# TheRealOrange/icer_compression

Hardware: AMD Instinct MI355X
Metric: Mpixels/s encode (bit-exact), 4096x4096 gray (higher is better)
Workload: dtype int16

## Files before the change

### icer_compression_amd/csrc/api.hip

```cpp
#include <hip/hip_runtime.h>

#include <algorithm>
#include <atomic>
#include <map>
#include <memory>
#include <mutex>
#include <thread>
#include <sched.h>
#include <time.h>
#include <stdarg.h>
#include <stdio.h>
#include <stdlib.h>
#include <string.h>
#include <string>
#include <vector>

#include "../../include/icer_hip.h"
#include "kernels.hpp"
#include "launch_plan.hpp"
#include "subband_gain.hpp"

using namespace icer;

namespace {
// ... 425 lines not shown
    return hipSuccess;
}
const char *pool_compute_level() { const char *v = getenv("ICER_HIP_COMPUTE_LEVEL"); return v ? v : "low"; }

#ifndef ICER_LONE_PAD_BYTES
#define ICER_LONE_PAD_BYTES 12288
#endif
constexpr int kLonePadBytes = ICER_LONE_PAD_BYTES;
static_assert(kUnitWavesSmall == 8 && kUnitWavesLarge == 11, "launch_plan.hpp names the pipeline's shapes by these wave counts");

int enqueue_budget_tail(icerx_encoder *e, const EncodeCall &c)
{
    const Budget &b = *c.budget;
    const uint32_t n_units = (uint32_t)e->plan.units.size();
    const size_t off_pitch = (size_t)e->max_frames * n_units, curve_pitch = (size_t)n_units + 1u;
    hipLaunchKernelGGL(budget_search_kernel, dim3(b.n), dim3(64 * kBudgetWaves), 0, c.stream, e->curve.p, e->curve.p + (size_t)e->max_frames * curve_pitch,
                       e->curve_head.p, n_units, (uint32_t)b.n_frames, b.budgets, (uint64_t)c.quota, e->unit_bits.p, e->final_order.p, e->skip(0), e->units.p,
                       e->final_off.p, off_pitch, reinterpret_cast<unsigned long long *>(c.d_sizes), c.d_rcs, b.d_at_cap, b.d_dist, b.d_equiv, b.d_threshold,
                       b.d_total, e->bound_ovf(), e->budget_state.p);
    hipLaunchKernelGGL(gather_ladder_kernel, dim3(n_units, b.n_frames), dim3(256), 0, c.stream, e->slots.p, e->plan.slot_bytes, e->units.p, n_units,
                       e->unit_bits.p, e->final_off.p, off_pitch, (uint32_t)b.n, c.d_out, c.out_stride, (uint32_t)b.n_frames);
    HIP_TRY(hipGetLastError());
    return 0;
}

int enqueue_part(icerx_encoder *e, const LaunchPlan &lp, int part, bool timed, const EncodeCall &c, bool clear_bound)
{
    const PartPlan &pp = lp.part[part];
    const int f0 = pp.f0, n_frames = pp.n_frames;
    const uint16_t *const d_frames = c.d_frames; uint8_t *const d_out = c.d_out; int32_t *const d_rcs = c.d_rcs;
    unsigned long long *const d_sizes = reinterpret_cast<unsigned long long *>(c.d_sizes);
    const size_t quota = c.quota, out_stride = c.out_stride;
    const hipStream_t st = c.stream; const Ladder *const ladder = c.ladder; const Target *const target = c.target; const Budget *const budget = c.budget;
    const Roi *const roi = c.roi;
    const bool energy = target || budget;
    const bool progressive = lp.progressive, use_wg = lp.use_wg, split = pp.split, hybrid = pp.hybrid;
    const size_t W = e->w, H = e->h, plane = W * H;
    const int C = e->channels, P = n_frames * C;
    const uint32_t n_units = (uint32_t)e->plan.units.size();
    int *dwt_ovf = e->dwt_ovf(f0), *mean_ovf = e->mean_ovf(f0), *skip = e->skip(f0), *bound_ovf = e->bound_ovf();
    int16_t *const coef = e->coef.p + (size_t)f0 * C * plane, *const tmp = e->tmp.p + (size_t)f0 * C * plane;
    unsigned long long *const sums = e->sums.p + (size_t)f0 * C;
    uint16_t *const means = e->means.p + (size_t)f0 * C;
    uint8_t *const sig = e->sig.p + (size_t)f0 * e->plan.sig_bytes;
    uint32_t *const sig_hist = e->sig_hist.p + (size_t)f0 * e->plan.n_families * 16;
    uint8_t *const route_buf = e->route.p + (size_t)f0 * n_units;
    uint32_t *const route_list = e->route_list.p + 2 * (size_t)f0 * n_units,        *const route_ctl = e->route_ctl.p + 4 * (size_t)part;
    uint8_t *const slots = e->slots.p + (size_t)f0 * e->plan.slot_bytes;
    uint32_t *const unit_bits = e->unit_bits.p + (size_t)f0 * n_units, *const done_bytes = e->done_bytes.p + (size_t)f0 * n_units;
    uint64_t *const final_off = e->final_off.p + (size_t)f0 * n_units;
    const size_t sub_entries = e->plan.sub_entries;
    if (split && (e->snaps.ensure((size_t)e->max_frames * sub_entries * kMaxSnaps) || e->snap_valid.ensure((size_t)e->max_frames * sub_entries * kMaxSnaps) ||
                  e->sub_recs.ensure((size_t)e->max_frames * sub_entries))) return ICER_FATAL_ERROR;
    {
        ClearList cl;
        const char *bad = nullptr;
        auto clear = [&](const char *what, void *ptr, size_t bytes) { if (!bad && !cl.add(ptr, bytes)) bad = what; };
        if (f0 == 0 && n_frames == e->max_frames && clear_bound) clear("frame flags", e->flags.p, e->flags.n * sizeof(int));
        else {
            clear("transform flags", dwt_ovf, (size_t)P * sizeof(int)); clear("mean flags", mean_ovf, (size_t)P * sizeof(int)); clear("skip flags", skip, (size_t)n_frames * sizeof(int));
            if (clear_bound) clear("slot bound flag", bound_ovf, sizeof(int));
        }
        clear("LL sums", sums, (size_t)P * sizeof(unsigned long long));
        if (progressive) clear("unit byte counts", done_bytes, (size_t)n_frames * n_units * 4);
        if (hybrid) { clear("chunk histograms", sig_hist, (size_t)n_frames * e->plan.n_families * 16 * sizeof(uint32_t)); clear("route list cursor", route_ctl, 4 * sizeof(uint32_t)); }
        if (split) { clear("snapshot flags", e->snap_valid.p, (size_t)n_frames * sub_entries * kMaxSnaps * sizeof(uint32_t)); clear("sub-range records", e->sub_recs.p, (size_t)n_frames * sub_entries * sizeof(SubRecord)); }
        if (bad) { set_error("enqueue: the clear kernel cannot take the %s range (%d ranges queued)", bad, cl.n); return ICER_FATAL_ERROR; }
        launch_clears(cl, st);
    }
    if (timed && e->timing) HIP_TRY(hipEventRecord(e->ev[0], st));

    size_t cw = W, ch = H;
    launch_dwt(e, d_frames, n_frames, st, e->sample_bits, dwt_ovf, &cw, &ch, coef, tmp);
    if (timed && e->timing) HIP_TRY(hipEventRecord(e->ev[1], st));

    const uint32_t llw = (uint32_t)cw, llh = (uint32_t)ch;
    unsigned sum_blocks = (llw * llh + 255) / 256;
    if (sum_blocks > 64) sum_blocks = 64;
    hipLaunchKernelGGL(ll_sum_kernel, dim3(sum_blocks, P), dim3(256), 0, st, reinterpret_cast<const uint16_t *>(coef),
                       plane, (uint32_t)W, llw, llh, sums, e->sample_bits == 8 ? 0xFFu : 0xFFFFu);
    hipLaunchKernelGGL(ll_mean_kernel, dim3((P + 63) / 64), dim3(64), 0, st, sums, (uint32_t)P, llw * llh,
                       means, mean_ovf, e->sample_bits);
    hipLaunchKernelGGL(frame_status_kernel, dim3((n_frames + 63) / 64), dim3(64), 0, st, dwt_ovf, mean_ovf, C, n_frames, skip);
    hipLaunchKernelGGL(finalize_ll_kernel, dim3((llw + 63u) / 64u, (llh + 3u) / 4u, P), dim3(256), 0, st,
                       reinterpret_cast<uint16_t *>(coef), plane, (uint32_t)W, llw, llh, means, skip, C, e->sample_bits);
    if (timed && e->timing) HIP_TRY(hipEventRecord(e->ev[2], st));
    if (e->coef_ready && f0 == 0) HIP_TRY(hipEventRecord(e->coef_ready, st));

    const int n_planes = e->sample_bits == 8 ? kPlanes8 : kPlanes;
    const size_t ev_frame_bytes = (size_t)n_planes * e->plan.sig_bytes * 64u;
    {
        hipLaunchKernelGGL(family_events_kernel, dim3((unsigned)(e->plan.sig_blocks.size() / 2), n_frames), dim3(256), 0, st,
                           reinterpret_cast<const uint16_t *>(coef), plane, (uint32_t)W, C, e->units.p, e->sig_blocks.p, skip, sig,
                           e->plan.sig_bytes, hybrid ? sig_hist : nullptr, e->plan.n_families,
                           use_wg ? nullptr : e->events.p + (size_t)f0 * ev_frame_bytes, ev_frame_bytes, (uint32_t)n_planes);
    }
    const uint8_t *route = nullptr;
    if (hybrid) {
        hipLaunchKernelGGL(route_units_kernel, dim3((unsigned)((n_units + 255) / 256), n_frames), dim3(256), 0, st, e->units.p, n_units, sig_hist, e->plan.n_families,
                           pp.route_percent, 16u, route_buf, route_list, route_ctl, kNoSplitPercent, (uint32_t)n_frames * n_units, kListHeavyMin);
        route = route_buf;
        HIP_TRY(hipEventRecord(e->fork[part], st));
        HIP_TRY(hipStreamWaitEvent(e->side_stream, e->fork[part], 0));
#define ICER_LAUNCH_LIST(I, NS)                                                                                                          \
        hipLaunchKernelGGL((code_units_list_kernel<I>), dim3(pp.list_grid), dim3(64 * NS::kWgWaves), sizeof(NS::Shared), e->side_stream, \
                           reinterpret_cast<const uint16_t *>(coef), plane, (uint32_t)W, (uint32_t)H, C, e->units.p, n_units,     \
                           e->tables.p, means, skip, slots, e->plan.slot_bytes, unit_bits, sig,                     \
                           e->plan.sig_bytes, route_list, route_ctl, e->prof.p ? e->prof.p + kProfWgsOffset : nullptr, (uint32_t)n_frames * n_units)
        if (pp.list == ListKernel::One) ICER_LAUNCH_LIST(WgOne, wg1); else if (pp.list == ListKernel::Four) ICER_LAUNCH_LIST(WgFour, wg4); else ICER_LAUNCH_LIST(WgSmall, wgs);
#undef ICER_LAUNCH_LIST
        HIP_TRY(hipEventRecord(e->join[part], e->side_stream));
    }
    const uint32_t tgt_planes = (uint32_t)n_planes;
    unsigned long long *const dist = energy ? e->dist.p + (size_t)f0 * e->plan.n_families * (tgt_planes + 1u) : nullptr;
    auto launch_energy = [&](hipStream_t es) -> int {
        HIP_TRY(hipMemsetAsync(dist, 0, (size_t)n_frames * e->plan.n_families * (tgt_planes + 1u) * sizeof(unsigned long long), es));
        hipLaunchKernelGGL(family_energy_kernel, dim3((unsigned)(e->plan.sig_blocks.size() / 2), n_frames), dim3(64 * kEnergyWaves), 0, es,
                           reinterpret_cast<const uint16_t *>(coef), plane, (uint32_t)W, C, e->units.p, e->sig_blocks.p, dist, e->plan.n_families, tgt_planes);
        return 0;
    };
    if (energy && e->side_stream) {
        HIP_TRY(hipEventRecord(e->energy_fork[part], st));
        HIP_TRY(hipStreamWaitEvent(e->side_stream, e->energy_fork[part], 0));
        if (launch_energy(e->side_stream)) return ICER_FATAL_ERROR;
        HIP_TRY(hipEventRecord(e->energy_join[part], e->side_stream));
    }
    SplitLaunch sp;
    if (split) {
        sp.subs = e->subs.p; sp.launch = e->sub_order.p; sp.n_subs = pp.subs; sp.entries = (uint32_t)sub_entries;
        sp.snaps = e->snaps.p; sp.snap_valid = e->snap_valid.p; sp.recs = e->sub_recs.p;
    }
    uint32_t fail_inject = ~0u;
    if (Tuning &t = e->tuning; t.fail_calls > 0 && !use_wg && t.fail_frame >= f0 && t.fail_frame < f0 + n_frames && t.fail_unit < (int)n_units) {
        fail_inject = ((uint32_t)(t.fail_frame - f0) << 20) | (uint32_t)t.fail_unit;
        t.fail_calls--;
    }
    if (!use_wg) {
        const dim3 pipe_grid = pp.position_major ? dim3((unsigned)((n_units + sp.n_subs) * (unsigned)n_frames), 1) : dim3(n_units + sp.n_subs, n_frames);
// ... 1279 lines not shown
```

### icer_compression_amd/csrc/events.hpp

```cpp
#pragma once
#include "icer_tables.hpp"
#include "wave.hpp"

namespace icer {

constexpr uint32_t kEvNone = 14u, kEvUncoded = 15u;

ICER_HD uint32_t ev_ctx_plain(uint32_t h, uint32_t v, uint32_t d)
{
    if (h == 2) return 8;
    if (h == 1) return (v == 0) ? (d < 2 ? 5 + d : 7u) : 7u;
    if (v == 0) return d > 2 ? 2u : d;
    return 2 + v;
}
ICER_HD uint32_t ev_ctx_hh(uint32_t hv, uint32_t d)
{
    if (d >= 3) return 8;
    const uint32_t k = hv > 2 ? 2u : hv;
    if (d == 0) return k;
    if (d == 1) return 3 + k;
    return hv == 0 ? 6u : 7u;
}
ICER_HD uint32_t ev_ctx_entry(bool is_hh, uint32_t i)
{
    return is_hh ? ev_ctx_hh(i / 5u, i % 5u) : ev_ctx_plain(i / 15u, (i / 5u) % 3u, i % 5u);
}

struct PixelLens {
    uint32_t mag;
    uint32_t msb;
    uint32_t aW, aE, aN, aS, aNW, aNE, aSW, aSE;
    uint32_t neg;
    uint32_t t;
};

ICER_HD uint32_t ev_len(uint32_t v) { const uint32_t m = v & 0x7FFFu; return m ? 32u - (uint32_t)__builtin_clz(m) : 0u; }

ICER_HD PixelLens pixel_lens(uint32_t vC, uint32_t vW, uint32_t vE, uint32_t vN, uint32_t vS, uint32_t vNW, uint32_t vNE, uint32_t vSW, uint32_t vSE)
{
    PixelLens L;
    const uint32_t lc = ev_len(vC);
    L.mag = vC & 0x7FFFu;
    L.msb = lc ? lc - 1u : 0u;
    L.aW = ev_len(vW); L.aN = ev_len(vN); L.aNW = ev_len(vNW); L.aNE = ev_len(vNE);
    const uint32_t lE = ev_len(vE), lS = ev_len(vS), lSW = ev_len(vSW), lSE = ev_len(vSE);
    L.aE = lE ? lE - 1u : 0u; L.aS = lS ? lS - 1u : 0u; L.aSW = lSW ? lSW - 1u : 0u; L.aSE = lSE ? lSE - 1u : 0u;
    L.neg = ((vW >> 15) & 1u) | (((vE >> 15) & 1u) << 1) | (((vN >> 15) & 1u) << 2) | (((vS >> 15) & 1u) << 3) | (((vC >> 15) & 1u) << 4);
    uint32_t t = lc;
    t = L.aW > t ? L.aW : t; t = L.aN > t ? L.aN : t; t = L.aNW > t ? L.aNW : t; t = L.aNE > t ? L.aNE : t;
    t = L.aE > t ? L.aE : t; t = L.aS > t ? L.aS : t; t = L.aSW > t ? L.aSW : t; t = L.aSE > t ? L.aSE : t;
    L.t = t;
    return L;
}

ICER_HD uint32_t event_byte(const PixelLens &L, uint32_t p, bool is_hl, bool is_hh, const uint8_t *ctx_tab)
{
    const uint32_t sW = L.aW > p, sE = L.aE > p, sN = L.aN > p, sS = L.aS > p;
    uint32_t hh = sW + sE, vv = sN + sS;
    const uint32_t dd = (uint32_t)(L.aNW > p) + (uint32_t)(L.aNE > p) + (uint32_t)(L.aSW > p) + (uint32_t)(L.aSE > p);
    const uint32_t up = L.msb > p ? L.msb - p : 0u, cat = up > 3u ? 3u : up;
    const uint32_t bit = (L.mag >> p) & 1u;
    uint32_t A = (L.neg & sW) | ((L.neg >> 1) & sE), B = ((L.neg >> 2) & sN) | ((L.neg >> 3) & sS);
    if (is_hl) { uint32_t x = hh; hh = vv; vv = x; x = A; A = B; B = x; }
    const uint32_t c0 = ctx_tab[is_hh ? (hh + vv) * 5u + dd : (hh * 3u + vv) * 5u + dd];
    const uint32_t ctx = cat == 0u ? c0 : cat == 1u ? (hh + vv == 0u ? 9u : 10u) : cat == 2u ? 11u : kEvUncoded;
    const uint32_t s2 = ((A & 1u) << 1) | ((A ^ B) & 1u);
    const uint32_t bit2 = (A ^ (L.neg >> 4)) & 1u;
    return ctx | (bit << 4) | (s2 << 5) | (bit2 << 7);
}

ICER_HD size_t ev_offset(uint32_t p, size_t chunks_per_frame, uint32_t chunk_off, uint32_t j) { return ((size_t)p * chunks_per_frame + chunk_off + j) * 64u; }

}
```

### icer_compression_amd/csrc/kernels.hpp

```cpp
#pragma once
#include <hip/hip_runtime.h>

#include "assemble_core.hpp"
#include "assemble_ladder.hpp"
#include "roi_core.hpp"
#include "coder_core.hpp"
#include "distortion_core.hpp"
#include "budget_core.hpp"
#include "coder_wg.hpp"
#include "coder_wg_small.hpp"
#include "dwt_tile.hpp"
#include "events.hpp"
#include "plan.hpp"

namespace icer {

__global__ void __launch_bounds__(kTileThreads)
dwt_tile_kernel(DwtStageArgs a, size_t src_plane, size_t coef_plane, size_t ll_plane, int *__restrict__ ovf)
{
    __shared__ union { DwtTileShared gen; DwtFastShared fast; } u;
    a.src += blockIdx.z * src_plane;
    a.coef += blockIdx.z * coef_plane;
    a.ll += blockIdx.z * ll_plane;
    const int tx = blockIdx.x, ty = blockIdx.y, t = threadIdx.x;
// ... 6 lines not shown
        __syncthreads();
        o |= dwt_fast_cols_step2(u.fast, a, tx, ty, t);
        if (o) atomicOr(&ovf[blockIdx.z], 1);
        return;
    }
    DwtTileShared &sh = u.gen;
    dwt_tile_load(sh, a, tx, ty, t);
    __syncthreads();
    bool o = dwt_tile_rows_step1(sh, a, tx, ty, t);
    __syncthreads();
    o |= dwt_tile_rows_step2(sh, a, tx, ty, t);
    __syncthreads();
    o |= dwt_tile_cols_step1(sh, a, tx, ty, t);
    __syncthreads();
    o |= dwt_tile_cols_step2(sh, a, tx, ty, t);
    if (o) atomicOr(&ovf[blockIdx.z], 1);
}

__global__ void __launch_bounds__(256)
ll_sum_kernel(const uint16_t *__restrict__ coef, size_t plane, uint32_t stride, uint32_t llw, uint32_t llh,
              unsigned long long *__restrict__ sums, uint32_t mask)
{
    const uint16_t *p = coef + blockIdx.y * plane;
    const uint32_t n = llw * llh;
    unsigned long long acc = 0;
    for (uint32_t i = blockIdx.x * 256 + threadIdx.x; i < n; i += gridDim.x * 256) {
        const uint32_t r = i / llw, c = i - r * llw;
        acc += p[(size_t)r * stride + c] & mask;
    }
    for (int o = 32; o > 0; o >>= 1) acc += __shfl_down(acc, o);
    if ((threadIdx.x & 63) == 0 && acc) atomicAdd(&sums[blockIdx.y], acc);
}

__global__ void ll_mean_kernel(const unsigned long long *__restrict__ sums, uint32_t n_planes, uint32_t ll_count,
                               uint16_t *__restrict__ means, int *__restrict__ mean_ovf, int sample_bits)
{
    const uint32_t p = blockIdx.x * blockDim.x + threadIdx.x;
    if (p >= n_planes) return;
    const uint16_t m = sample_bits == 8 ? (uint16_t)(uint8_t)(sums[p] / ll_count) : (uint16_t)(sums[p] / ll_count);
    means[p] = m;
    mean_ovf[p] = m > (sample_bits == 8 ? 127 : 32767) ? 1 : 0;
}

__global__ void __launch_bounds__(256)
finalize_ll_kernel(uint16_t *__restrict__ coef, size_t plane, uint32_t w, uint32_t llw, uint32_t llh,
                   const uint16_t *__restrict__ means, const int *__restrict__ frame_skip, int channels, int sample_bits)
{
    const uint32_t c = blockIdx.x * 64 + (threadIdx.x & 63), r = blockIdx.y * 4 + (threadIdx.x >> 6);
    if (c >= llw || r >= llh) return;
    if (frame_skip[blockIdx.z / channels]) return;
    uint16_t *q = coef + blockIdx.z * plane + (size_t)r * w + c;
    const int16_t v = (int16_t)((int16_t)*q - (int16_t)means[blockIdx.z]);
    *q = (uint16_t)to_coder_word(v, sample_bits);
}

struct SplitLaunch {
    const SubDesc *subs = nullptr;
    const uint32_t *launch = nullptr;
    uint32_t n_subs = 0;
    uint32_t entries = 0;
    Snapshot *snaps = nullptr;
    uint32_t *snap_valid = nullptr;
    SubRecord *recs = nullptr;
};

constexpr uint8_t kRoutePipeline = 0, kRouteWindows = 1, kRouteNoSplit = 2;

template <int WAVES, int OCC, int LDS_PAD>
__global__ void __launch_bounds__(64 * WAVES, OCC)
code_units_kernel(const uint16_t *__restrict__ coef, size_t plane, uint32_t img_w, uint32_t img_h, int channels,
                  const UnitDesc *__restrict__ units, const uint32_t *__restrict__ work_order, uint32_t n_units,
                  const CoderTables *__restrict__ tables, const uint16_t *__restrict__ means,
                  const int *__restrict__ frame_skip, uint8_t *__restrict__ slots,
                  size_t slot_frame_stride, uint32_t *__restrict__ unit_bits, uint64_t *__restrict__ timers,
                  uint32_t *__restrict__ done_bytes, uint64_t early_quota, const uint8_t *__restrict__ route, SplitLaunch sp, uint32_t n_frames_1d,
                  const uint8_t *__restrict__ ev, size_t ev_frame_stride, const uint8_t *__restrict__ sig, size_t sig_frame_stride,
                  uint32_t fail_inject)
{
    __shared__ CoderShared s;
    if constexpr (LDS_PAD > 0) {
        __shared__ uint32_t lds_pad[LDS_PAD / 4];
        if (early_quota == ~0ull) lds_pad[threadIdx.x] = 1u;
    }
    uint32_t frame = blockIdx.y, lpos = blockIdx.x;
    if (gridDim.y == 1u && n_frames_1d > 1u) {
        position_major(blockIdx.x, n_units + sp.n_subs, n_frames_1d, &frame, &lpos);
        if (frame >= n_frames_1d) return;
    }
    const uint32_t entry = sp.n_subs ? sp.launch[lpos] : (work_order ? work_order[lpos] : lpos);
    const bool sub_block = sp.n_subs != 0u && (entry >> 31) != 0u;
    const SubDesc sd = sub_block ? sp.subs[entry & 0x7FFFFFFFu] : SubDesc{};
    const uint32_t ui = sub_block ? sd.unit : entry;
    const uint8_t rt = route ? route[(size_t)frame * n_units + ui] : kRoutePipeline;
    if (rt == kRouteWindows) return;
    if (sub_block && rt != kRoutePipeline) return;
#ifdef ICER_PHASE_TIMERS
    uint64_t *trace = (timers && frame == 0 && lpos < (uint32_t)kTraceUnits) ? timers + 9 * 32 + 4 * lpos : nullptr;
    if (trace && threadIdx.x == 0) {
        trace[0] = wall_clock64();
        trace[2] = (uint64_t)__builtin_amdgcn_s_getreg((31 << 11) | 4) | ((uint64_t)__builtin_amdgcn_s_getreg((3 << 11) | 20) << 32);
        trace[3] = entry;
    }
    if (timers && frame == 0 && lpos == 0 && (threadIdx.x & 63) == 0)
        timers[9 * 32 + 4 * kTraceUnits + (threadIdx.x >> 6)] = (uint64_t)__builtin_amdgcn_s_getreg((31 << 11) | 4);
#endif
    const uint32_t wave = (uint32_t)__builtin_amdgcn_readfirstlane((int)(threadIdx.x >> 6));
// ... 169 lines not shown
            }
        }
#ifdef ICER_PHASE_TIMERS
        if (trace && (threadIdx.x & 63) == 0) trace[1] = wall_clock64();
#endif
    }
}

constexpr uint32_t kSpliceWaves = 4;
__global__ void __launch_bounds__(64 * kSpliceWaves)
splice_units_kernel(const UnitDesc *__restrict__ units, uint32_t n_units, const CoderTables *__restrict__ tables,
                    const uint16_t *__restrict__ means, const int *__restrict__ frame_skip, int channels, uint32_t img_w, uint32_t img_h,
                    uint8_t *__restrict__ slots, size_t slot_frame_stride, uint32_t *__restrict__ unit_bits,
                    const uint8_t *__restrict__ route, SplitLaunch sp)
{
    struct SpliceShared { uint32_t crc_tab[256]; struct { uint32_t x2n[32]; } tab; uint32_t parts[kSpliceWaves]; };
    __shared__ SpliceShared s;
    const uint32_t frame = blockIdx.y, ui = blockIdx.x;
    const UnitDesc u = units[ui];
    if (u.n_sub <= 1u || frame_skip[frame]) return;
    if (route && route[(size_t)frame * n_units + ui] != kRoutePipeline) return;
    build_crc_table(s);
    if (threadIdx.x < 32) s.tab.x2n[threadIdx.x] = tables->x2n[threadIdx.x];
    __syncthreads();
    uint8_t *fs = slots + (size_t)frame * slot_frame_stride;
    uint32_t *slot_words = reinterpret_cast<uint32_t *>(fs + u.slot_off);
    uint32_t *words[kMaxSubs];
    words[0] = slot_words + kHeaderBytes / 4;
    for (uint32_t i = 1; i < u.n_sub; i++) words[i] = reinterpret_cast<uint32_t *>(fs + sp.subs[u.sub_first + i - 1u].slot_off);
    const size_t e = (size_t)frame * sp.entries + u.sub_entry;
    __builtin_amdgcn_fence(__ATOMIC_ACQUIRE, "agent");
    const uint32_t wv = threadIdx.x >> 6;
    const uint32_t bits = splice_unit_wave(u.n_sub, sp.recs + e, sp.snaps + e * kMaxSnaps, words, u.cap_words, wv, kSpliceWaves);
    if (bits != kUnitTooBig && bits != kUnitFailed) {
        __threadfence();
        FinishArgs f;
        f.slot_words = slot_words;
        f.bits = bits;
        f.mean = means[(size_t)frame * channels + u.chan];
        f.level = u.level; f.subband = u.subband; f.seg = u.seg; f.lsb = u.lsb; f.chan = u.chan;
        f.image_w = img_w; f.image_h = img_h;
        __syncthreads();
        finish_unit_wave(s, f, wv, kSpliceWaves, s.parts);
    }
    if (threadIdx.x == 0) unit_bits[(size_t)frame * n_units + ui] = bits;
}

__global__ void __launch_bounds__(256)
family_events_kernel(const uint16_t *__restrict__ coef, size_t plane, uint32_t img_w, int channels,
                     const UnitDesc *__restrict__ units, const uint32_t *__restrict__ blocks, const int *__restrict__ frame_skip,
                     uint8_t *__restrict__ sig, size_t sig_frame_stride, uint32_t *__restrict__ hist, uint32_t n_families,
                     uint8_t *__restrict__ ev, size_t ev_frame_stride, uint32_t n_planes)
{
    __shared__ uint8_t ctx_tab[48];
    const UnitDesc u = units[blocks[2u * blockIdx.x]];
    const uint32_t frame = blockIdx.y, nchunks = (u.w * u.h + 63u) / 64u, first = blocks[2u * blockIdx.x + 1u] * 64u;
    if (frame_skip[frame]) return;
    const bool is_hl = u.subband == kHL, is_hh = u.subband == kHH;
    if (ev) {
        if (threadIdx.x < 45u) ctx_tab[threadIdx.x] = (uint8_t)ev_ctx_entry(is_hh, threadIdx.x);
        __syncthreads();
    }
    const uint16_t *seg = coef + ((size_t)frame * channels + u.chan) * plane + (size_t)u.y0 * img_w + u.x0;
    uint8_t *out = sig + (size_t)frame * sig_frame_stride + u.sig_off;
    uint8_t *evf = ev ? ev + (size_t)frame * ev_frame_stride : nullptr;
    const uint32_t wave = threadIdx.x >> 6, lane = threadIdx.x & 63u;
    const uint32_t sw = u.w, sh = u.h, npix = sw * sh;
    uint32_t j = first + wave * 16u;
    uint32_t np = j * 64u + lane;
    uint32_t r = np / sw, c = np - r * sw;
    uint32_t mine = 0;
    for (uint32_t i = 0; i < 16u && j < nchunks; i++, j++) {
        const bool in_ = np < npix;
        const uint32_t r_ = in_ ? r : 0u, c_ = in_ ? c : 0u;
        const bool hasW_ = c_ > 0, hasE_ = c_ + 1 < sw, hasN_ = r_ > 0, hasS_ = r_ + 1 < sh;
        const uint32_t cW_ = hasW_ ? c_ - 1u : c_, cE_ = hasE_ ? c_ + 1u : c_;
        const uint16_t *pC_ = seg + (size_t)r_ * img_w;
        const uint16_t *pN_ = hasN_ ? pC_ - img_w : pC_, *pS_ = hasS_ ? pC_ + img_w : pC_;
        const uint32_t vC = pC_[c_], vW = pC_[cW_], vE = pC_[cE_], vN = pN_[c_], vNW = pN_[cW_], vNE = pN_[cE_];
        const uint32_t vS = pS_[c_], vSW = pS_[cW_], vSE = pS_[cE_];
        const PixelLens L = pixel_lens(vC, hasW_ ? vW : 0u, hasE_ ? vE : 0u, hasN_ ? vN : 0u, hasS_ ? vS : 0u, (hasN_ && hasW_) ? vNW : 0u,
                                       (hasN_ && hasE_) ? vNE : 0u, (hasS_ && hasW_) ? vSW : 0u, (hasS_ && hasE_) ? vSE : 0u);
        uint32_t tmax = 0;
        for (uint32_t step = 8u; step; step >>= 1) tmax += __ballot(in_ && L.t >= tmax + step) ? step : 0u;
        const bool partial = __ballot(!in_) != 0ull;
        if (lane == 0u) out[j] = (uint8_t)(partial ? 255u : tmax);
        mine += (!partial && lane == tmax) ? 1u : 0u;
        if (evf) {
            const uint32_t top = partial ? n_planes : (tmax < n_planes ? tmax : n_planes);
            for (uint32_t p = 0; p < top; p++)
                evf[ev_offset(p, sig_frame_stride, u.sig_off, j) + lane] = (uint8_t)(in_ ? event_byte(L, p, is_hl, is_hh, ctx_tab) : kEvNone);
        }
        np += 64u;
        c += 64u;
        if (sw >= 64u) { if (c >= sw) { c -= sw; r++; } }
        else { r = np / sw; c = np - r * sw; }
    }
    if (hist && lane < 16u && mine) atomicAdd(&hist[((size_t)frame * n_families + u.family) * 16u + lane], mine);
}

__global__ void __launch_bounds__(256)
route_units_kernel(const UnitDesc *__restrict__ units, uint32_t n_units, const uint32_t *__restrict__ hist, uint32_t n_families,
                   uint32_t percent, uint32_t min_chunks, uint8_t *__restrict__ route, uint32_t *__restrict__ list,
                   uint32_t *__restrict__ list_ctl, uint32_t nosplit_percent, uint32_t list_cap, uint32_t heavy_min)
{
    const uint32_t ui = blockIdx.x * 256u + threadIdx.x, frame = blockIdx.y;
    const bool valid = ui < n_units;
    const UnitDesc u = units[valid ? ui : 0u];
    const uint32_t nchunks = (u.w * u.h + 63u) / 64u;
    const uint32_t *h = hist + ((size_t)frame * n_families + u.family) * 16u;
    uint32_t total = 0;
    for (uint32_t v = 0; v < 16u; v++) total += v <= u.lsb ? h[v] : 0u;
    const bool windows = valid && nchunks >= min_chunks && total * 100u >= percent * nchunks;
    if (valid) route[(size_t)frame * n_units + ui] = windows ? kRouteWindows : (total * 100u >= nosplit_percent * nchunks ? kRouteNoSplit : kRoutePipeline);
    const bool heavy = windows && nchunks - total >= heavy_min, light = windows && !heavy;
    const uint32_t lane = threadIdx.x & 63u;
    const uint64_t mh = __ballot(heavy), ml = __ballot(light);
    if (mh | ml) {
        const uint32_t nh = (uint32_t)__popcll(mh), nl = (uint32_t)__popcll(ml);
        uint32_t bh = 0, bl = 0;
        if (lane == 0u) {
            if (nh) bh = atomicAdd(&list_ctl[2], nh);
            if (nl) bl = atomicAdd(&list_ctl[3], nl);
            atomicAdd(&list_ctl[0], nh + nl);
        }
        bh = (uint32_t)__shfl((int)bh, 0); bl = (uint32_t)__shfl((int)bl, 0);
        const uint32_t rh = (uint32_t)__builtin_amdgcn_mbcnt_hi((uint32_t)(mh >> 32), __builtin_amdgcn_mbcnt_lo((uint32_t)mh, 0u));
        const uint32_t rl = (uint32_t)__builtin_amdgcn_mbcnt_hi((uint32_t)(ml >> 32), __builtin_amdgcn_mbcnt_lo((uint32_t)ml, 0u));
        if (heavy) list[list_cap + bh + rh] = frame * n_units + ui;
        if (light) list[bl + rl] = frame * n_units + ui;
    }
}

struct WgLaunch {
    const uint16_t *coef; size_t plane; uint32_t img_w, img_h; int channels;
    const UnitDesc *units; uint32_t n_units; const uint16_t *means; const int *frame_skip; uint8_t *slots;
    size_t slot_frame_stride; uint32_t *unit_bits; uint64_t *timers; uint32_t *done_bytes; uint64_t early_quota;
    const uint8_t *sig; size_t sig_frame_stride;
};
struct WgFull {
    using Shared = wg::Shared; using UnitArgs = wg::UnitArgs; using Wave = wg::Wave;
    static constexpr uint32_t kWaves = wg::kWgWaves;
    static __device__ __forceinline__ void init(Shared &s, const UnitArgs &a) { wg::unit_state_init(s, a); }
    static __device__ __forceinline__ bool spent(const UnitArgs &a) { return wg::quota_already_spent(a); }
// ... 100 lines not shown
                     const int *__restrict__ frame_skip, uint8_t *__restrict__ slots,
                     size_t slot_frame_stride, uint32_t *__restrict__ unit_bits, uint64_t *__restrict__ timers,
                     uint32_t *__restrict__ done_bytes, uint64_t early_quota,
                     const uint8_t *__restrict__ sig, size_t sig_frame_stride)
{
    extern __shared__ __attribute__((aligned(16))) unsigned char wg_lds[];
    typename I::Shared &s = *reinterpret_cast<typename I::Shared *>(wg_lds);
    const uint32_t ui = work_order ? work_order[blockIdx.x] : blockIdx.x;
    wg_shared_tables<I>(s, tables);
    const WgLaunch L{coef, plane, img_w, img_h, channels, units, n_units, means, frame_skip, slots, slot_frame_stride, unit_bits, timers,
                     done_bytes, early_quota, sig, sig_frame_stride};
    wg_code_one_unit<I>(s, L, blockIdx.y, ui);
}

template <class I>
__global__ void __launch_bounds__(64 * I::kWaves)
code_units_list_kernel(const uint16_t *__restrict__ coef, size_t plane, uint32_t img_w, uint32_t img_h, int channels,
                       const UnitDesc *__restrict__ units, uint32_t n_units,
                       const CoderTables *__restrict__ tables, const uint16_t *__restrict__ means,
                       const int *__restrict__ frame_skip, uint8_t *__restrict__ slots,
                       size_t slot_frame_stride, uint32_t *__restrict__ unit_bits,
                       const uint8_t *__restrict__ sig, size_t sig_frame_stride,
                       const uint32_t *__restrict__ list, uint32_t *__restrict__ list_ctl, uint64_t *__restrict__ timers, uint32_t list_cap)
{
    extern __shared__ __attribute__((aligned(16))) unsigned char wg_lds[];
    typename I::Shared &s = *reinterpret_cast<typename I::Shared *>(wg_lds);
    __shared__ uint32_t next_entry;
    wg_shared_tables<I>(s, tables);
    const WgLaunch L{coef, plane, img_w, img_h, channels, units, n_units, means, frame_skip, slots, slot_frame_stride, unit_bits, timers,
                     nullptr, 0ull, sig, sig_frame_stride};
    const uint32_t count = list_ctl[0], n_heavy = list_ctl[2];
    for (;;) {
        __syncthreads();
        if (threadIdx.x == 0) next_entry = atomicAdd(&list_ctl[1], 1u);
        __syncthreads();
        const uint32_t at = next_entry;
        if (at >= count) break;
        const uint32_t e = at < n_heavy ? list[list_cap + at] : list[at - n_heavy];
#ifdef ICER_PHASE_TIMERS
        const uint64_t t_start = wall_clock64();
#endif
        wg_code_one_unit<I>(s, L, e / n_units, e % n_units);
#ifdef ICER_PHASE_TIMERS
        if (timers && threadIdx.x == 0 && at < (uint32_t)kListTrace && e < n_units) {
            const UnitDesc &ud = units[e];
            uint64_t *tr = timers + 9 * 32 + 4 * at;
            tr[0] = t_start; tr[1] = wall_clock64(); tr[2] = blockIdx.x | ((uint64_t)e << 32);
            tr[3] = (uint64_t)ud.lsb | ((uint64_t)ud.level << 8) | ((uint64_t)ud.subband << 16) | ((uint64_t)ud.seg << 24) | ((uint64_t)((ud.w * ud.h + 63u) / 64u) << 32);
        }
#endif
    }
}

__global__ void __launch_bounds__(64)
scan_kernel(const uint32_t *__restrict__ unit_bits, const uint32_t *__restrict__ final_order, uint32_t n_units,
            uint64_t quota, const int *__restrict__ frame_skip, uint64_t *__restrict__ final_off,
            unsigned long long *__restrict__ sizes, int32_t *__restrict__ rcs, const UnitDesc *__restrict__ units,
            int *__restrict__ bound_overflow)
{
    const uint32_t frame = blockIdx.x;
    uint64_t *foff = final_off + (size_t)frame * n_units;
    if (frame_skip[frame]) {
        for (uint32_t i = threadIdx.x; i < n_units; i += 64) foff[i] = ~0ull;
        if (threadIdx.x == 0) { sizes[frame] = 0; rcs[frame] = kIntegerOverflow; }
        return;
    }
    const uint32_t *bits = unit_bits + (size_t)frame * n_units;
    {
        int failed = 0;
        for (uint32_t i = threadIdx.x; i < n_units; i += 64) failed |= bits[i] == kUnitFailed;
        if (__ballot(failed)) {
            for (uint32_t i = threadIdx.x; i < n_units; i += 64) foff[i] = ~0ull;
            if (threadIdx.x == 0) { sizes[frame] = 0; rcs[frame] = kFatalError; atomicOr(bound_overflow, 2); }
            return;
        }
    }
    uint32_t kept;
    uint64_t used;
    const int rc = scan_frame_wave(bits, final_order, n_units, quota, foff, &kept, &used);
    if (kept < n_units && threadIdx.x == 0 && bits[kept] == kUnitTooBig && units[kept].cap_is_bound)
        atomicOr(bound_overflow, 1);
    if (threadIdx.x == 0) { sizes[frame] = used; rcs[frame] = rc; }
}

__global__ void __launch_bounds__(256)
gather_kernel(const uint8_t *__restrict__ slots, size_t slot_frame_stride, const UnitDesc *__restrict__ units,
              uint32_t n_units, const uint32_t *__restrict__ unit_bits, const uint64_t *__restrict__ final_off,
              uint8_t *__restrict__ out, size_t out_stride)
{
    const uint32_t frame = blockIdx.y, ui = blockIdx.x;
    const uint64_t off = final_off[(size_t)frame * n_units + ui];
    if (off == ~0ull) return;
    const uint32_t len = kHeaderBytes + ((unit_bits[(size_t)frame * n_units + ui] + 7u) >> 3);
    const uint8_t *src = slots + (size_t)frame * slot_frame_stride + units[ui].slot_off;
    uint8_t *dst = out + (size_t)frame * out_stride + off;
    const uint32_t mis = (uint32_t)((4u - ((uintptr_t)dst & 3u)) & 3u);
    const uint32_t head = mis < len ? mis : len;
    if (threadIdx.x < head) dst[threadIdx.x] = src[threadIdx.x];
    const uint32_t body_words = (len - head) >> 2;
    const uint32_t *sw = reinterpret_cast<const uint32_t *>(src);
    uint32_t *dw = reinterpret_cast<uint32_t *>(dst + head);
    const uint32_t shift = head * 8;
    for (uint32_t i = threadIdx.x; i < body_words; i += 256) {
        const uint32_t lo = sw[i];
        uint32_t v = lo;
        if (shift) v = (lo >> shift) | (sw[i + 1] << (32 - shift));
        dw[i] = v;
    }
    const uint32_t done = head + body_words * 4;
    if (threadIdx.x < len - done) dst[done + threadIdx.x] = src[done + threadIdx.x];
}


__global__ void __launch_bounds__(64)
scan_ladder_kernel(const uint32_t *__restrict__ unit_bits, const uint32_t *__restrict__ final_order, uint32_t n_units,
                   LadderQuotas quotas, const int *__restrict__ frame_skip, uint64_t *__restrict__ final_off, size_t off_pitch,
                   unsigned long long *__restrict__ sizes, int32_t *__restrict__ rcs, uint32_t pitch, const UnitDesc *__restrict__ units,
                   int *__restrict__ bound_overflow)
{
    const uint32_t frame = blockIdx.x, q = blockIdx.y;
    const size_t row = (size_t)q * pitch + frame;
    const uint32_t flags = scan_ladder_wave(unit_bits + (size_t)frame * n_units, final_order, n_units, quotas.q[q], frame_skip[frame], units,
                                            final_off + (size_t)q * off_pitch + (size_t)frame * n_units, sizes + row, rcs + row);
    if (flags && threadIdx.x == 0) atomicOr(bound_overflow, (int)flags);
}

__global__ void __launch_bounds__(256)
gather_ladder_kernel(const uint8_t *__restrict__ slots, size_t slot_frame_stride, const UnitDesc *__restrict__ units,
                     uint32_t n_units, const uint32_t *__restrict__ unit_bits, const uint64_t *__restrict__ final_off, size_t off_pitch,
                     uint32_t n_q, uint8_t *__restrict__ out, size_t out_stride, uint32_t pitch)
{
    const uint32_t frame = blockIdx.y, ui = blockIdx.x;
    const uint64_t *offs = final_off + (size_t)frame * n_units + ui;
// ... 138 lines not shown
```

Measured before the change: 3411.

## Fuse LL mean kernels, precompute event bitplanes, shuffle neighbors, stage scan in LDS

New measurement: 3420 (median of 6 runs). No clear change (+0.3%).

```diff
diff --git a/icer_compression_amd/csrc/api.hip b/icer_compression_amd/csrc/api.hip
--- a/icer_compression_amd/csrc/api.hip
+++ b/icer_compression_amd/csrc/api.hip
@@ -501,6 +501,9 @@
     const size_t sub_entries = e->plan.sub_entries;
     if (split && (e->snaps.ensure((size_t)e->max_frames * sub_entries * kMaxSnaps) || e->snap_valid.ensure((size_t)e->max_frames * sub_entries * kMaxSnaps) ||
                   e->sub_recs.ensure((size_t)e->max_frames * sub_entries))) return ICER_FATAL_ERROR;
+    size_t ll_count = 0;
+    { size_t lw = W, lh = H; for (int s = 0; s < e->stages; s++) { lw = (lw + 1) / 2; lh = (lh + 1) / 2; } ll_count = lw * lh; }
+    const bool ll_fused = ll_count <= kLlFusedMax;
     {
         ClearList cl;
         const char *bad = nullptr;
@@ -510,7 +513,7 @@
             clear("transform flags", dwt_ovf, (size_t)P * sizeof(int)); clear("mean flags", mean_ovf, (size_t)P * sizeof(int)); clear("skip flags", skip, (size_t)n_frames * sizeof(int));
             if (clear_bound) clear("slot bound flag", bound_ovf, sizeof(int));
         }
-        clear("LL sums", sums, (size_t)P * sizeof(unsigned long long));
+        if (!ll_fused) clear("LL sums", sums, (size_t)P * sizeof(unsigned long long));
         if (progressive) clear("unit byte counts", done_bytes, (size_t)n_frames * n_units * 4);
         if (hybrid) { clear("chunk histograms", sig_hist, (size_t)n_frames * e->plan.n_families * 16 * sizeof(uint32_t)); clear("route list cursor", route_ctl, 4 * sizeof(uint32_t)); }
         if (split) { clear("snapshot flags", e->snap_valid.p, (size_t)n_frames * sub_entries * kMaxSnaps * sizeof(uint32_t)); clear("sub-range records", e->sub_recs.p, (size_t)n_frames * sub_entries * sizeof(SubRecord)); }
@@ -524,15 +527,20 @@
     if (timed && e->timing) HIP_TRY(hipEventRecord(e->ev[1], st));
 
     const uint32_t llw = (uint32_t)cw, llh = (uint32_t)ch;
-    unsigned sum_blocks = (llw * llh + 255) / 256;
-    if (sum_blocks > 64) sum_blocks = 64;
-    hipLaunchKernelGGL(ll_sum_kernel, dim3(sum_blocks, P), dim3(256), 0, st, reinterpret_cast<const uint16_t *>(coef),
-                       plane, (uint32_t)W, llw, llh, sums, e->sample_bits == 8 ? 0xFFu : 0xFFFFu);
-    hipLaunchKernelGGL(ll_mean_kernel, dim3((P + 63) / 64), dim3(64), 0, st, sums, (uint32_t)P, llw * llh,
-                       means, mean_ovf, e->sample_bits);
-    hipLaunchKernelGGL(frame_status_kernel, dim3((n_frames + 63) / 64), dim3(64), 0, st, dwt_ovf, mean_ovf, C, n_frames, skip);
-    hipLaunchKernelGGL(finalize_ll_kernel, dim3((llw + 63u) / 64u, (llh + 3u) / 4u, P), dim3(256), 0, st,
-                       reinterpret_cast<uint16_t *>(coef), plane, (uint32_t)W, llw, llh, means, skip, C, e->sample_bits);
+    if (ll_fused) {
+        hipLaunchKernelGGL(ll_mean_finalize_kernel, dim3(n_frames), dim3(kLlFusedThreads), 0, st, reinterpret_cast<uint16_t *>(coef), plane, (uint32_t)W,
+                           llw, llh, C, e->sample_bits, dwt_ovf, means, mean_ovf, skip);
+    } else {
+        unsigned sum_blocks = (llw * llh + 255) / 256;
+        if (sum_blocks > 64) sum_blocks = 64;
+        hipLaunchKernelGGL(ll_sum_kernel, dim3(sum_blocks, P), dim3(256), 0, st, reinterpret_cast<const uint16_t *>(coef),
+                           plane, (uint32_t)W, llw, llh, sums, e->sample_bits == 8 ? 0xFFu : 0xFFFFu);
+        hipLaunchKernelGGL(ll_mean_kernel, dim3((P + 63) / 64), dim3(64), 0, st, sums, (uint32_t)P, llw * llh,
+                           means, mean_ovf, e->sample_bits);
+        hipLaunchKernelGGL(frame_status_kernel, dim3((n_frames + 63) / 64), dim3(64), 0, st, dwt_ovf, mean_ovf, C, n_frames, skip);
+        hipLaunchKernelGGL(finalize_ll_kernel, dim3((llw + 63u) / 64u, (llh + 3u) / 4u, P), dim3(256), 0, st,
+                           reinterpret_cast<uint16_t *>(coef), plane, (uint32_t)W, llw, llh, means, skip, C, e->sample_bits);
+    }
     if (timed && e->timing) HIP_TRY(hipEventRecord(e->ev[2], st));
     if (e->coef_ready && f0 == 0) HIP_TRY(hipEventRecord(e->coef_ready, st));
 
diff --git a/icer_compression_amd/csrc/events.hpp b/icer_compression_amd/csrc/events.hpp
--- a/icer_compression_amd/csrc/events.hpp
+++ b/icer_compression_amd/csrc/events.hpp
@@ -69,6 +69,52 @@
     return ctx | (bit << 4) | (s2 << 5) | (bit2 << 7);
 }
 
+struct EventPlanes {
+    uint32_t h0, h1, v0, v1, d0, d1, d2, c0, c1, mag, sx, sa, sb;
+};
+
+ICER_HD uint32_t ev_mask(uint32_t a) { return (1u << a) - 1u; }
+
+ICER_HD uint32_t ev_planes_entry(bool is_hh, uint32_t i)
+{
+    const uint32_t h = i & 3u, v = (i >> 2) & 3u, d = (i >> 4) & 7u, cat = (i >> 7) & 3u;
+    if (cat == 3u) return kEvUncoded;
+    if (cat == 2u) return 11u;
+    if (cat == 1u) return h + v == 0u ? 9u : 10u;
+    if (h > 2u || v > 2u || d > 4u) return 0u;
+    return ev_ctx_entry(is_hh, is_hh ? (h + v) * 5u + d : (h * 3u + v) * 5u + d);
+}
+
+ICER_HD EventPlanes event_planes(const PixelLens &L, bool is_hl)
+{
+    const uint32_t mW = ev_mask(L.aW), mE = ev_mask(L.aE), mN = ev_mask(L.aN), mS = ev_mask(L.aS);
+    const uint32_t mNW = ev_mask(L.aNW), mNE = ev_mask(L.aNE), mSW = ev_mask(L.aSW), mSE = ev_mask(L.aSE);
+    uint32_t h0 = mW ^ mE, h1 = mW & mE, v0 = mN ^ mS, v1 = mN & mS;
+    const uint32_t s1 = mNW ^ mNE, k1 = mNW & mNE, s2 = mSW ^ mSE, k2 = mSW & mSE;
+    uint32_t A = ((L.neg & 1u) ? mW : 0u) | ((L.neg & 2u) ? mE : 0u), B = ((L.neg & 4u) ? mN : 0u) | ((L.neg & 8u) ? mS : 0u);
+    if (is_hl) { uint32_t x = h0; h0 = v0; v0 = x; x = h1; h1 = v1; v1 = x; x = A; A = B; B = x; }
+    const uint32_t g1 = ev_mask(L.msb), g2 = g1 >> 1, g3 = g1 >> 2;
+    EventPlanes E;
+    E.h0 = h0; E.h1 = h1 << 1; E.v0 = v0 << 2; E.v1 = v1 << 3;
+    E.d0 = (s1 ^ s2) << 4; E.d1 = (k1 ^ k2 ^ (s1 & s2)) << 5; E.d2 = (k1 & k2) << 6;
+    E.c0 = (g1 ^ g2 ^ g3) << 7; E.c1 = g2 << 8;
+    E.mag = L.mag << 9;
+    E.sx = (A ^ B) << 10; E.sa = A << 11; E.sb = (A ^ ((L.neg & 16u) ? ~0u : 0u)) << 12;
+    return E;
+}
+
+ICER_HD uint32_t event_planes_byte(const EventPlanes &E, uint32_t p, const uint8_t *tab)
+{
+    const uint32_t one = 1u << p;
+    uint32_t x = E.h0 & one;
+    x |= E.h1 & (one << 1); x |= E.v0 & (one << 2); x |= E.v1 & (one << 3);
+    x |= E.d0 & (one << 4); x |= E.d1 & (one << 5); x |= E.d2 & (one << 6);
+    x |= E.c0 & (one << 7); x |= E.c1 & (one << 8); x |= E.mag & (one << 9);
+    x |= E.sx & (one << 10); x |= E.sa & (one << 11); x |= E.sb & (one << 12);
+    x >>= p;
+    return tab[x & 511u] | ((x >> 5) & 0xF0u);
+}
+
 ICER_HD size_t ev_offset(uint32_t p, size_t chunks_per_frame, uint32_t chunk_off, uint32_t j) { return ((size_t)p * chunks_per_frame + chunk_off + j) * 64u; }
 
 }
diff --git a/icer_compression_amd/csrc/kernels.hpp b/icer_compression_amd/csrc/kernels.hpp
--- a/icer_compression_amd/csrc/kernels.hpp
+++ b/icer_compression_amd/csrc/kernels.hpp
@@ -82,6 +82,47 @@
     uint16_t *q = coef + blockIdx.z * plane + (size_t)r * w + c;
     const int16_t v = (int16_t)((int16_t)*q - (int16_t)means[blockIdx.z]);
     *q = (uint16_t)to_coder_word(v, sample_bits);
+}
+
+constexpr uint32_t kLlFusedMax = 65536u, kLlFusedThreads = 1024u;
+__global__ void __launch_bounds__(kLlFusedThreads)
+ll_mean_finalize_kernel(uint16_t *__restrict__ coef, size_t plane, uint32_t stride, uint32_t llw, uint32_t llh, int channels, int sample_bits,
+                        const int *__restrict__ dwt_ovf, uint16_t *__restrict__ means, int *__restrict__ mean_ovf, int *__restrict__ skip)
+{
+    __shared__ uint32_t part[kLlFusedThreads / 64u];
+    const uint32_t frame = blockIdx.x, n = llw * llh, mask = sample_bits == 8 ? 0xFFu : 0xFFFFu;
+    int bad = 0;
+    for (int ch = 0; ch < channels; ch++) {
+        const size_t pl = (size_t)frame * channels + ch;
+        const uint16_t *p = coef + pl * plane;
+        uint32_t acc = 0;
+        for (uint32_t i = threadIdx.x; i < n; i += kLlFusedThreads) {
+            const uint32_t r = i / llw, c = i - r * llw;
+            acc += p[(size_t)r * stride + c] & mask;
+        }
+        for (int o = 32; o > 0; o >>= 1) acc += __shfl_down(acc, o);
+        if ((threadIdx.x & 63u) == 0u) part[threadIdx.x >> 6] = acc;
+        __syncthreads();
+        uint32_t sum = 0;
+        for (uint32_t i = 0; i < kLlFusedThreads / 64u; i++) sum += part[i];
+        const uint16_t m = sample_bits == 8 ? (uint16_t)(uint8_t)(sum / n) : (uint16_t)(sum / n);
+        const int o = m > (sample_bits == 8 ? 127 : 32767) ? 1 : 0;
+        if (threadIdx.x == 0) { means[pl] = m; mean_ovf[pl] = o; }
+        bad |= o | dwt_ovf[pl];
+        __syncthreads();
+    }
+    if (threadIdx.x == 0) skip[frame] = bad;
+    if (bad) return;
+    for (int ch = 0; ch < channels; ch++) {
+        const size_t pl = (size_t)frame * channels + ch;
+        uint16_t *p = coef + pl * plane;
+        const int16_t m = (int16_t)means[pl];
+        for (uint32_t i = threadIdx.x; i < n; i += kLlFusedThreads) {
+            const uint32_t r = i / llw, c = i - r * llw;
+            uint16_t *q = p + (size_t)r * stride + c;
+            *q = (uint16_t)to_coder_word((int16_t)((int16_t)*q - m), sample_bits);
+        }
+    }
 }
 
 struct SplitLaunch {
@@ -357,13 +398,13 @@
                      uint8_t *__restrict__ sig, size_t sig_frame_stride, uint32_t *__restrict__ hist, uint32_t n_families,
                      uint8_t *__restrict__ ev, size_t ev_frame_stride, uint32_t n_planes)
 {
-    __shared__ uint8_t ctx_tab[48];
+    __shared__ uint8_t ev_tab[512];
     const UnitDesc u = units[blocks[2u * blockIdx.x]];
     const uint32_t frame = blockIdx.y, nchunks = (u.w * u.h + 63u) / 64u, first = blocks[2u * blockIdx.x + 1u] * 64u;
     if (frame_skip[frame]) return;
     const bool is_hl = u.subband == kHL, is_hh = u.subband == kHH;
     if (ev) {
-        if (threadIdx.x < 45u) ctx_tab[threadIdx.x] = (uint8_t)ev_ctx_entry(is_hh, threadIdx.x);
+        for (uint32_t i = threadIdx.x; i < 512u; i += 256u) ev_tab[i] = (uint8_t)ev_planes_entry(is_hh, i);
         __syncthreads();
     }
     const uint16_t *seg = coef + ((size_t)frame * channels + u.chan) * plane + (size_t)u.y0 * img_w + u.x0;
@@ -371,6 +412,7 @@
     uint8_t *evf = ev ? ev + (size_t)frame * ev_frame_stride : nullptr;
     const uint32_t wave = threadIdx.x >> 6, lane = threadIdx.x & 63u;
     const uint32_t sw = u.w, sh = u.h, npix = sw * sh;
+    const bool wide = sw >= 64u;
     uint32_t j = first + wave * 16u;
     uint32_t np = j * 64u + lane;
     uint32_t r = np / sw, c = np - r * sw;
@@ -382,8 +424,21 @@
         const uint32_t cW_ = hasW_ ? c_ - 1u : c_, cE_ = hasE_ ? c_ + 1u : c_;
         const uint16_t *pC_ = seg + (size_t)r_ * img_w;
         const uint16_t *pN_ = hasN_ ? pC_ - img_w : pC_, *pS_ = hasS_ ? pC_ + img_w : pC_;
-        const uint32_t vC = pC_[c_], vW = pC_[cW_], vE = pC_[cE_], vN = pN_[c_], vNW = pN_[cW_], vNE = pN_[cE_];
-        const uint32_t vS = pS_[c_], vSW = pS_[cW_], vSE = pS_[cE_];
+        const uint32_t vC = pC_[c_], vN = pN_[c_], vS = pS_[c_];
+        uint32_t vW, vE, vNW, vNE, vSW, vSE;
+        if (wide) {
+            uint32_t xC = 0, xN = 0, xS = 0;
+            if (lane == 0u || lane == 63u) {
+                const uint32_t cX_ = lane == 0u ? cW_ : cE_;
+                xC = pC_[cX_]; xN = pN_[cX_]; xS = pS_[cX_];
+            }
+            const uint32_t cn = vC | (vN << 16);
+            const uint32_t cnW = __shfl_up(cn, 1), sW = __shfl_up(vS, 1), cnE = __shfl_down(cn, 1), sE = __shfl_down(vS, 1);
+            vW = lane == 0u ? xC : cnW & 0xFFFFu; vNW = lane == 0u ? xN : cnW >> 16; vSW = lane == 0u ? xS : sW;
+            vE = lane == 63u ? xC : cnE & 0xFFFFu; vNE = lane == 63u ? xN : cnE >> 16; vSE = lane == 63u ? xS : sE;
+        } else {
+            vW = pC_[cW_]; vE = pC_[cE_]; vNW = pN_[cW_]; vNE = pN_[cE_]; vSW = pS_[cW_]; vSE = pS_[cE_];
+        }
         const PixelLens L = pixel_lens(vC, hasW_ ? vW : 0u, hasE_ ? vE : 0u, hasN_ ? vN : 0u, hasS_ ? vS : 0u, (hasN_ && hasW_) ? vNW : 0u,
                                        (hasN_ && hasE_) ? vNE : 0u, (hasS_ && hasW_) ? vSW : 0u, (hasS_ && hasE_) ? vSE : 0u);
         uint32_t tmax = 0;
@@ -393,8 +448,11 @@
         mine += (!partial && lane == tmax) ? 1u : 0u;
         if (evf) {
             const uint32_t top = partial ? n_planes : (tmax < n_planes ? tmax : n_planes);
-            for (uint32_t p = 0; p < top; p++)
-                evf[ev_offset(p, sig_frame_stride, u.sig_off, j) + lane] = (uint8_t)(in_ ? event_byte(L, p, is_hl, is_hh, ctx_tab) : kEvNone);
+            if (top) {
+                const EventPlanes E = event_planes(L, is_hl);
+                for (uint32_t p = 0; p < top; p++)
+                    evf[ev_offset(p, sig_frame_stride, u.sig_off, j) + lane] = (uint8_t)(in_ ? event_planes_byte(E, p, ev_tab) : kEvNone);
+            }
         }
         np += 64u;
         c += 64u;
@@ -601,6 +659,8 @@
     }
 }
 
+constexpr uint32_t kScanStageUnits = 4096u;
+constexpr uint32_t kScanStageBatch = 8u;
 __global__ void __launch_bounds__(64)
 scan_kernel(const uint32_t *__restrict__ unit_bits, const uint32_t *__restrict__ final_order, uint32_t n_units,
             uint64_t quota, const int *__restrict__ frame_skip, uint64_t *__restrict__ final_off,
@@ -614,10 +674,31 @@
         if (threadIdx.x == 0) { sizes[frame] = 0; rcs[frame] = kIntegerOverflow; }
         return;
     }
+    __shared__ uint32_t lds_bits[kScanStageUnits], lds_order[kScanStageUnits];
     const uint32_t *bits = unit_bits + (size_t)frame * n_units;
+    const bool staged = n_units <= kScanStageUnits;
     {
         int failed = 0;
-        for (uint32_t i = threadIdx.x; i < n_units; i += 64) failed |= bits[i] == kUnitFailed;
+        if (staged) {
+            for (uint32_t base = 0; base < n_units; base += 64u * kScanStageBatch) {
+                uint32_t b[kScanStageBatch], o[kScanStageBatch];
+#pragma unroll
+                for (uint32_t k = 0; k < kScanStageBatch; k++) {
+                    const uint32_t i = base + 64u * k + threadIdx.x;
+                    b[k] = i < n_units ? bits[i] : 0u;
+                    o[k] = i < n_units ? final_order[i] : 0u;
+                }
+#pragma unroll
+                for (uint32_t k = 0; k < kScanStageBatch; k++) {
+                    const uint32_t i = base + 64u * k + threadIdx.x;
+                    if (i < n_units) { lds_bits[i] = b[k]; lds_order[i] = o[k]; }
+                    failed |= b[k] == kUnitFailed;
+                }
+            }
+            __syncthreads();
+        } else {
+            for (uint32_t i = threadIdx.x; i < n_units; i += 64) failed |= bits[i] == kUnitFailed;
+        }
         if (__ballot(failed)) {
             for (uint32_t i = threadIdx.x; i < n_units; i += 64) foff[i] = ~0ull;
             if (threadIdx.x == 0) { sizes[frame] = 0; rcs[frame] = kFatalError; atomicOr(bound_overflow, 2); }
@@ -626,8 +707,9 @@
     }
     uint32_t kept;
     uint64_t used;
-    const int rc = scan_frame_wave(bits, final_order, n_units, quota, foff, &kept, &used);
-    if (kept < n_units && threadIdx.x == 0 && bits[kept] == kUnitTooBig && units[kept].cap_is_bound)
+    const int rc = staged ? scan_frame_wave(lds_bits, lds_order, n_units, quota, foff, &kept, &used)
+                          : scan_frame_wave(bits, final_order, n_units, quota, foff, &kept, &used);
+    if (kept < n_units && threadIdx.x == 0 && (staged ? lds_bits[kept] : bits[kept]) == kUnitTooBig && units[kept].cap_is_bound)
         atomicOr(bound_overflow, 1);
     if (threadIdx.x == 0) { sizes[frame] = used; rcs[frame] = rc; }
 }
```
